# ut-amrl/vision_slam_frontend

Hardware: AMD Instinct MI355X
Metric: stereo frames/s (640x480, 2000 kp/frame) (higher is better)
Workload: dtype u8

## Files before the change

include/vsf.h:

```cpp
#ifndef VSF_H_
#define VSF_H_

#include <stddef.h>
#include <stdint.h>

#ifdef __cplusplus
extern "C" {
#endif

#define VSF_VERSION 2
#define VSF_DESC_BYTES 32
#define VSF_MAX_LEVELS 64

typedef enum {
  VSF_OK = 0,
  VSF_ERR_INVALID_ARG = 1,
  VSF_ERR_CAPACITY = 2,
  VSF_ERR_HIP = 3,
  VSF_ERR_UNSUPPORTED = 4,
  VSF_ERR_NO_DEVICE = 5
} vsf_status;

typedef struct {
  float x, y;
// ... 240 lines not shown


vsf_status vsf_debug_png_encode_header(int width, int height, int channels, uint8_t* out, size_t cap, size_t* n_bytes);
vsf_status vsf_debug_png_encode_cpu(const uint8_t* src, int width, int height, int channels, size_t src_row_stride, uint8_t* out,
                                    size_t cap, size_t* n_bytes);

vsf_status vsf_debug_jpeg_encode_header(int width, int height, int channels, int quality, uint8_t* out, size_t cap,
                                        size_t* n_bytes);

vsf_status vsf_debug_inject_hip_error(vsf_ctx* ctx, int code);
vsf_status vsf_debug_level_image(vsf_ctx* ctx, int image, int level, int blurred, uint8_t* out, size_t ostride);
vsf_status vsf_debug_fast_candidates(vsf_ctx* ctx, int image, int level, vsf_keypoint* kp_out, int cap,
                                     int* n_out);
vsf_status vsf_debug_fast_work(const vsf_params* p, int orb, int nms, uint32_t* words, int cap, int* n_words, int* n_full,
                               int32_t* levels_out, int level_cap);
vsf_status vsf_debug_level_keypoints(vsf_ctx* ctx, int image, int level, vsf_keypoint* kp_out, int cap,
                                     int* n_out);
vsf_status vsf_debug_retain_best(vsf_ctx* ctx, uint32_t* key_bits, uint32_t* ids, int n, int n_points, int use_lds,
                                 int mode, int* n_out);
vsf_status vsf_debug_sort_trim(vsf_ctx* ctx, const vsf_dmatch* matches, int n_lists, int n, float best_percent,
                               int serial, uint64_t* pairs_out, int32_t* counts_out);

vsf_status vsf_debug_jpeg_serial(vsf_ctx* ctx, int on);

#define VSF_STAGE_COUNT 8
enum { VSF_STAGE_PYRAMID = 0, VSF_STAGE_FAST, VSF_STAGE_SELECT, VSF_STAGE_BLUR, VSF_STAGE_DESCRIBE, VSF_STAGE_KNN2,
       VSF_STAGE_RATIO, VSF_STAGE_TAIL  };
vsf_status vsf_profile_enable(vsf_ctx* ctx, int on);
vsf_status vsf_profile_read(vsf_ctx* ctx, double* ms_total, int64_t* launches, int reset);
const char* vsf_stage_name(int stage);
// ... 9 lines not shown
```

vision_slam_frontend_amd/capi.py:

```python
from __future__ import annotations

import ctypes as C
from pathlib import Path

import numpy as np

_PKG = Path(__file__).resolve().parent
LIB_PATH = _PKG / "libvsf_hip.so"

KEYPOINT_DTYPE = np.dtype([("x", "<f4"), ("y", "<f4"), ("size", "<f4"), ("angle", "<f4"), ("response", "<f4"),
                           ("octave", "<i4"), ("class_id", "<i4")])
DMATCH_DTYPE = np.dtype([("queryIdx", "<i4"), ("trainIdx", "<i4"), ("imgIdx", "<i4"), ("distance", "<f4")])
VISION_FEATURE_DTYPE = np.dtype([("feature_idx", "<u8"), ("pixel", "<f4", (2,)), ("point3d", "<f4", (3,))])
FEATURE_MATCH_DTYPE = np.dtype([("feature_idx_initial", "<u8"), ("feature_idx_current", "<u8")])
assert VISION_FEATURE_DTYPE.itemsize == 28 and FEATURE_MATCH_DTYPE.itemsize == 16
DESC_BYTES = 32
PAYLOAD_MAGIC = 0x31465356

VSF_OK, VSF_ERR_INVALID_ARG, VSF_ERR_CAPACITY, VSF_ERR_HIP, VSF_ERR_UNSUPPORTED, VSF_ERR_NO_DEVICE = range(6)

EXPORTS = [
    "vsf_params_default", "vsf_params_set_ratio", "vsf_create", "vsf_destroy", "vsf_status_string",
    "vsf_last_hip_error", "vsf_get_params", "vsf_set_stream", "vsf_sync", "vsf_level_info", "vsf_extract",
    "vsf_fast_detect", "vsf_knn2_hamming", "vsf_get_matches", "vsf_extract_pair", "vsf_get_matches_multi", "vsf_extract_batch_dev", "vsf_match_batch_dev",
    "vsf_stereo_batch_dev", "vsf_set_lanes", "vsf_set_pipeline", "vsf_set_blur_overlap", "vsf_set_fast_resident", "vsf_get_fast_resident", "vsf_remove_ambig_stereo_batch_dev", "vsf_feature_matches_batch_dev", "vsf_bayer_bg_to_gray_batch_dev", "vsf_debug_level_image", "vsf_debug_fast_candidates", "vsf_debug_fast_work", "vsf_debug_level_keypoints",
    "vsf_algorithmic_bytes_per_image", "vsf_pyramid_pixels", "vsf_profile_enable", "vsf_profile_read",
    "vsf_stage_name", "vsf_debug_retain_best", "vsf_debug_sort_trim", "vsf_stereo_residuals_batch_dev", "vsf_stereo_thresholds_dev",
    "vsf_stereo_filter_batch_dev", "vsf_vision_features_batch_dev", "vsf_packed_outputs_capacity",
    "vsf_pack_outputs_dev", "vsf_observe_capacity", "vsf_observe_stereo", "vsf_observe_submit", "vsf_observe_collect", "vsf_observe_reset",
    "vsf_observe_configure", "vsf_observe_collect_view", "vsf_observe_stats", "vsf_observe_poll", "vsf_debug_jpeg_serial",
    "vsf_jpeg_decode_gray_batch", "vsf_png_decode_gray_batch", "vsf_imdecode_gray_batch", "vsf_tune_fast_resident", "vsf_set_option", "vsf_get_option", "vsf_debug_inject_hip_error", "vsf_comm_unique_id", "vsf_comm_create", "vsf_comm_destroy", "vsf_comm_info",
    "vsf_allgather_dev", "vsf_gather_payload_dev", "vsf_reserve", "vsf_set_input_event",
    "vsf_observe_set_debug_images", "vsf_observe_debug_view", "vsf_draw_canvases_dev", "vsf_draw_canvases",
    "vsf_observe_submit_compressed", "vsf_observe_stereo_compressed", "vsf_observe_set_compressed_cap",
    "vsf_observe_default_compressed_cap", "vsf_observe_compressed_slot_bytes", "vsf_observe_compressed_ring_bytes",
    "vsf_compressed_image_size", "vsf_observe_probe_compressed",
    "vsf_observe_set_debug_jpeg", "vsf_observe_debug_jpeg_view", "vsf_jpeg_encode_capacity", "vsf_jpeg_encode_batch_dev", "vsf_jpeg_encode", "vsf_debug_jpeg_encode_header",
    "vsf_png_encode_capacity", "vsf_png_encode_batch_dev", "vsf_png_encode", "vsf_debug_png_encode_header", "vsf_debug_png_encode_cpu", "vsf_observe_set_debug_png", "vsf_observe_debug_png_view",
]
(OPT_FAST_BOTH_MAX, OPT_SELECT_WIDE, OPT_PYRAMID_FEW, OPT_PYRAMID_CHAIN, OPT_PYRAMID_ROWS, OPT_SELECT_BIG_CLASS,
# ... 186 lines not shown
        L.vsf_observe_probe_compressed.argtypes = [vp, sz, i32, i32, sz, i32, ip]
        L.vsf_observe_set_debug_images.argtypes = [vp, i32]
        L.vsf_observe_debug_view.argtypes = [vp, C.c_int64, C.POINTER(vp), C.POINTER(vp)]
        L.vsf_observe_set_debug_jpeg.argtypes = [vp, i32]
        L.vsf_observe_debug_jpeg_view.argtypes = [vp, C.c_int64, C.POINTER(vp), C.POINTER(sz), C.POINTER(vp), C.POINTER(sz)]
        L.vsf_observe_set_debug_png.argtypes = [vp, i32]
        L.vsf_observe_debug_png_view.argtypes = [vp, C.c_int64, C.POINTER(vp), C.POINTER(sz), C.POINTER(vp), C.POINTER(sz)]
        L.vsf_draw_canvases_dev.argtypes = [vp, C.POINTER(VsfDrawCanvas), i32, vp, i32]
        L.vsf_draw_canvases.argtypes = [vp, C.POINTER(VsfDrawCanvas), i32, vp, i32]
        L.vsf_jpeg_decode_gray_batch.argtypes = [vp, vp, vp, i32, i32, i32, vp, sz, sz]
        L.vsf_png_decode_gray_batch.argtypes = [vp, vp, vp, i32, i32, i32, vp, sz, sz]
        L.vsf_imdecode_gray_batch.argtypes = [vp, vp, vp, i32, i32, i32, vp, sz, sz]
        L.vsf_debug_level_image.argtypes = [vp, i32, i32, i32, vp, sz]
        L.vsf_debug_fast_candidates.argtypes = [vp, i32, i32, vp, i32, ip]
        L.vsf_debug_fast_work.argtypes = [vp, i32, i32, vp, i32, ip, ip, vp, i32]
        L.vsf_debug_level_keypoints.argtypes = [vp, i32, i32, vp, i32, ip]
        L.vsf_algorithmic_bytes_per_image.argtypes = [vp]
        L.vsf_algorithmic_bytes_per_image.restype = C.c_uint64
        L.vsf_pyramid_pixels.argtypes = [vp]
        L.vsf_pyramid_pixels.restype = C.c_uint64
        L.vsf_debug_retain_best.argtypes = [vp, vp, vp, i32, i32, i32, i32, ip]
        L.vsf_profile_enable.argtypes = [vp, i32]
        L.vsf_profile_read.argtypes = [vp, C.POINTER(C.c_double), C.POINTER(C.c_int64), i32]
        L.vsf_stage_name.argtypes = [i32]
        L.vsf_stage_name.restype = C.c_char_p
        _lib = L
    return _lib


def _p(a):
# ... 518 lines not shown
```

vision_slam_frontend_amd/csrc/k_fast.hip:

```cpp
#include "vsf_gather.h"
#include <cstdlib>

#include "vsf_internal.h"

namespace {

typedef short v2s __attribute__((ext_vector_type(2)));
constexpr int SR = VSF_FAST_STRIP_ROWS;

struct FastArgs {
  const VsfLevel* levels;
  const uint32_t* units;
  int nwork_full;
  int nunits;
  const uint8_t* img0;
  size_t img0_stride;
  int img0_pitch;
  const uint8_t* pyr;
  uint32_t pyr_bytes;
  uint32_t* cand;
  uint32_t cand_entries;
  uint16_t* rowstart;
  int threshold;
  int nms;
};

__device__ __forceinline__ uint32_t wave_shr1(uint32_t v) {
  return (uint32_t)__builtin_amdgcn_update_dpp(0, (int)v, 0x138, 0xF, 0xF, true);
// ... 99 lines not shown

__device__ __forceinline__ ScoreRow make_score_row(v2s s02, v2s s13) {
  ScoreRow o;
  o.s02 = s02;
  o.s13 = s13;
  const v2s x = as_v2s(__builtin_amdgcn_alignbit(as_u32(s13), wave_shr1(as_u32(s13)), 16));
  const v2s y = as_v2s(__builtin_amdgcn_alignbit(wave_shl1(as_u32(s02)), as_u32(s02), 16));
  o.h2a = vmax(x, s13);
  o.h2b = vmax(s02, y);
  o.h3a = vmax3(x, s13, s02);
  o.h3b = vmax3(s02, y, s13);
  return o;
}

template <bool PACK, bool NMS>
__device__ __forceinline__ void fast_march_body(const FastArgs& a, int work, int image) {
  const int lane = threadIdx.x & 63;
  int level, band, strip, hl, nl, nrows0 = 0;
  bool valid = true, mixed = false, rim = false;
  VsfLevel L;
  if constexpr (PACK) {
    struct Item {
      uint32_t w[VSF_FAST_PACK_WORDS];
    };
    const Item P = uniform_copy(reinterpret_cast<const Item*>(a.units + a.nwork_full) + work);
    uint32_t w0 = P.w[4], w1 = P.w[5];
#pragma unroll
    for (int k = 1; k < VSF_FAST_PACK_SEGS; k++)
      if (k < (int)P.w[0] && lane >= (int)(P.w[5 + 2 * k] & 0xFFu)) w0 = P.w[4 + 2 * k], w1 = P.w[5 + 2 * k];
    nrows0 = (int)P.w[1];
    mixed = P.w[2] != 0u;
    rim = P.w[3] != 0u;
    level = (int)(w0 >> 24), band = (int)((w0 >> 16) & 0xFF), strip = (int)(w0 & 0x7FFF);
    hl = lane - (int)(w1 & 0xFFu);
    nl = (int)((w1 >> 8) & 0xFFu);
    valid = hl < nl;
    L = a.levels[level];
  } else {
    const uint32_t ud = uniform_copy(a.units + work);
    level = (int)(ud >> 24), band = (int)((ud >> 16) & 0xFF), strip = (int)(ud & 0x7FFF);
    L = uniform_copy(a.levels + level);
    hl = lane, nl = 64;
  }
  const int pitch = level == 0 ? a.img0_pitch : L.pitch, hrow = L.h;
  const uint8_t* src;
  uint32_t src_bytes;
  if constexpr (PACK) {
    const bool lvl0 = __builtin_amdgcn_readfirstlane(level) == 0;
    src = lvl0 ? a.img0 + (size_t)image * a.img0_stride : a.pyr + (size_t)image * a.pyr_bytes;
    src_bytes = lvl0 ? (uint32_t)(a.img0_pitch * __builtin_amdgcn_readfirstlane(hrow)) : a.pyr_bytes;
  } else {
    src = level == 0 ? a.img0 + (size_t)image * a.img0_stride : a.pyr + (size_t)image * a.pyr_bytes + L.offset;
    src_bytes = (uint32_t)(pitch * hrow);
  }
  const int t = a.threshold;
  const int offs = NMS ? max(t, 1) : t;
  const v2s toff = {(short)offs, (short)offs};
  const int bx0 = L.fast_a0 + VSF_FAST_BAND_COLS * band;
  const int c0 = bx0 - 4 + 4 * hl;
  const bool loadable = valid && c0 >= 0 && c0 + 3 < pitch;
  const int ys = L.y_lo + strip * SR;
  const int nrows = valid ? min(SR, L.y_hi - ys) : 0;
  if constexpr (!PACK) nrows0 = nrows;
  const int sx_lo = max(L.x_lo - 1, 3), sx_hi = min(L.x_hi + 1, L.w - 3);
  uint32_t sm02 = 0, sm13 = 0, em02 = 0, em13 = 0;
#pragma unroll
  for (int j = 0; j < 4; j++) {
    const int x = c0 + j;
    const uint32_t bit = 0xFFFFu << (16 * (j >> 1));
    const bool sc_ok = valid && ((hl >= 1 && hl <= nl - 2) || (hl == 0 && j == 3) || (hl == nl - 1 && j == 0)) &&
                       x >= sx_lo && x < sx_hi;
    const bool em_ok = valid && hl >= 1 && hl <= nl - 2 && x >= L.x_lo && x < L.x_hi && x < bx0 + VSF_FAST_BAND_COLS;
    if (j & 1) {
      if (sc_ok) sm13 |= bit;
      if (em_ok) em13 |= bit;
    } else {
      if (sc_ok) sm02 |= bit;
      if (em_ok) em02 |= bit;
    }
  }
  const int unit_local = strip * L.nbands + band;
  uint16_t* rs = a.rowstart + ((size_t)image * a.nunits + L.unit0 + unit_local) * VSF_FAST_RS_STRIDE;
  const int seg_cap = L.seg_cap;
  const __amdgpu_buffer_rsrc_t seg_rsrc =
      PACK ? __builtin_amdgcn_make_buffer_rsrc(a.cand + (size_t)image * a.cand_entries, 0, a.cand_entries * 4, 0x00020000)
           : __builtin_amdgcn_make_buffer_rsrc(a.cand + (size_t)image * a.cand_entries + L.cand_offset +
                                                   (size_t)unit_local * seg_cap,
                                               0, seg_cap * 4, 0x00020000);
  const uint32_t seg_off = PACK ? 4u * (L.cand_offset + (uint32_t)(unit_local * seg_cap)) : 0u;
  const __amdgpu_buffer_rsrc_t rs_rsrc = __builtin_amdgcn_make_buffer_rsrc(
      a.rowstart + (size_t)image * a.nunits * VSF_FAST_RS_STRIDE, 0, a.nunits * VSF_FAST_RS_STRIDE * 2, 0x00020000);
  const uint32_t rs_off = 2u * (uint32_t)((L.unit0 + unit_local) * VSF_FAST_RS_STRIDE);
  const bool rs_lane = PACK && valid && hl == 0;
  const int cfirst = lane - hl, cend = min(cfirst + nl, 64);
  const unsigned long long from_m = ~0ull << cfirst, cell_m = from_m & (cend >= 64 ? ~0ull : (1ull << cend) - 1ull);
  const uint32_t from_lo = (uint32_t)from_m, from_hi = (uint32_t)(from_m >> 32);
  const uint32_t cell_lo = (uint32_t)cell_m, cell_hi = (uint32_t)(cell_m >> 32);

  const __amdgpu_buffer_rsrc_t src_rsrc = __builtin_amdgcn_make_buffer_rsrc(const_cast<uint8_t*>(src), 0, src_bytes, 0x00020000);
  const uint32_t col_off = loadable ? (uint32_t)c0 : 0xFFFFFFF0u;
  const int qlo = 1 - ys, qhi = hrow - ys;
  const uint32_t rbase = loadable ? (level == 0 ? 0u : L.offset) + (uint32_t)(c0 + (ys - 1) * pitch) : 0x40000000u;
  auto load_row = [&](int q) -> uint32_t {
    if (PACK)
      return __builtin_amdgcn_raw_buffer_load_b32(src_rsrc, rbase + (uint32_t)__mul24(min(max(q, qlo), qhi), pitch), 0u,
                                                  0);
    const int yc = min(max(ys - 1 + q, 0), hrow - 1);
    return __builtin_amdgcn_raw_buffer_load_b32(src_rsrc, col_off, (uint32_t)(yc * pitch), 0);
// ... 2 lines not shown
  const unsigned long long scorable = __builtin_amdgcn_ballot_w64((sm02 | sm13) != 0u);
  const v2s zero2 = {0, 0};
  ScoreRow S0 = make_score_row(zero2, zero2), S1 = S0, S2 = S0;
  int count = 0;
  uint32_t my_rs = 0;
  const uint32_t yx0 = ((uint32_t)ys << 12) + (uint32_t)c0 + ((uint32_t)(NMS ? offs - 1 : 0) << 24);
  auto below = [&](unsigned long long b, int acc) -> int {
    if (PACK)
      return (int)__builtin_amdgcn_mbcnt_hi((uint32_t)(b >> 32) & from_hi,
                                            __builtin_amdgcn_mbcnt_lo((uint32_t)b & from_lo, (uint32_t)acc));
    return (int)__builtin_amdgcn_mbcnt_hi((uint32_t)(b >> 32), __builtin_amdgcn_mbcnt_lo((uint32_t)b, (uint32_t)acc));
  };
  auto in_cell = [&](unsigned long long b) -> int {
    if (PACK) return __popc((uint32_t)b & cell_lo) + __popc((uint32_t)(b >> 32) & cell_hi);
    return __popcll(b);
  };

  auto step = [&](int q, const RowP& R0, const RowP& R1, const RowP& R2, const RowP& R3, const RowP& R4,
                  const RowP& R5, RowP& R6, const ScoreRow& S_up, const ScoreRow& S_mid, ScoreRow& S_dn) {
    prep_row(R6);
    v2s s02 = zero2, s13 = zero2;
    const int sy = ys - 1 + q;
    const bool row_ok = sy >= 3 && sy < hrow - 3;
    const uint32_t far = max(__builtin_amdgcn_sad_u8(R0.d, R3.d, 0u), __builtin_amdgcn_sad_u8(R6.d, R3.d, 0u));
    unsigned long long want = __builtin_amdgcn_ballot_w64(far > (uint32_t)t) & scorable;
    if (PACK) {
      if (rim) want &= __builtin_amdgcn_ballot_w64(row_ok);
    } else {
      want &= row_ok ? ~0ull : 0ull;
    }
// ... 48 lines not shown
            if (k1) {
              if (!PACK || pos < seg_cap) __builtin_amdgcn_raw_buffer_store_b32(yx + 1, seg_rsrc, seg_off + 4u * (uint32_t)pos, 0, 0);
              ++pos;
            }
            if (k2) {
              if (!PACK || pos < seg_cap) __builtin_amdgcn_raw_buffer_store_b32(yx + 2, seg_rsrc, seg_off + 4u * (uint32_t)pos, 0, 0);
              ++pos;
            }
            if (k3) {
              if (!PACK || pos < seg_cap) __builtin_amdgcn_raw_buffer_store_b32(yx + 3, seg_rsrc, seg_off + 4u * (uint32_t)pos, 0, 0);
            }
            count += in_cell(b0) + in_cell(b1) + in_cell(b2) + in_cell(b3);
          }
        }
      }
      if (r + 1 < SR) {
        if (PACK) {
          if (rs_lane)
            __builtin_amdgcn_raw_buffer_store_b16((unsigned short)min(count, seg_cap), rs_rsrc, rs_off, 2u * (uint32_t)(r + 1), 0);
        } else {
          asm("s_mov_b32 m0, %2\n\ts_nop 0\n\tv_writelane_b32 %0, %1, m0" : "+v"(my_rs) : "s"(min(count, seg_cap)), "s"(r + 1));
        }
      }
    }
  };

  RowP A0, A1, A2, A3, A4, A5, A6, A7, A8;
  A0.d = load_row(-3), A1.d = load_row(-2), A2.d = load_row(-1), A3.d = load_row(0), A4.d = load_row(1), A5.d = load_row(2),
  A6.d = load_row(3), A7.d = load_row(4);
  prep_row(A0), prep_row(A1), prep_row(A2), prep_row(A3), prep_row(A4), prep_row(A5);
  const int qe = nrows0 + 1;
#define VSF_FAST_STEP(j, r0, r1, r2, r3, r4, r5, r6, ld, su, sm, sd) \
  if (q + (j) > qe) break;                                             \
  ld.d = load_row(q + (j) + 5);                                        \
  step(q + (j), r0, r1, r2, r3, r4, r5, r6, su, sm, sd);
  for (int q = 0;; q += 9) {
    VSF_FAST_STEP(0, A0, A1, A2, A3, A4, A5, A6, A8, S0, S1, S2)
    VSF_FAST_STEP(1, A1, A2, A3, A4, A5, A6, A7, A0, S1, S2, S0)
    VSF_FAST_STEP(2, A2, A3, A4, A5, A6, A7, A8, A1, S2, S0, S1)
    VSF_FAST_STEP(3, A3, A4, A5, A6, A7, A8, A0, A2, S0, S1, S2)
    VSF_FAST_STEP(4, A4, A5, A6, A7, A8, A0, A1, A3, S1, S2, S0)
    VSF_FAST_STEP(5, A5, A6, A7, A8, A0, A1, A2, A4, S2, S0, S1)
    VSF_FAST_STEP(6, A6, A7, A8, A0, A1, A2, A3, A5, S0, S1, S2)
    VSF_FAST_STEP(7, A7, A8, A0, A1, A2, A3, A4, A6, S1, S2, S0)
    VSF_FAST_STEP(8, A8, A0, A1, A2, A3, A4, A5, A7, S2, S0, S1)
  }
#undef VSF_FAST_STEP
  if (PACK) {
    if (rs_lane) {
      rs[0] = 0;
      rs[SR] = (uint16_t)min(count, seg_cap);
    }
  } else {
    if (hl < SR) rs[hl] = (uint16_t)my_rs;
    if (hl == 0) rs[SR] = (uint16_t)min(count, seg_cap);
  }
}

template <bool PACK, bool NMS>
__global__ __launch_bounds__(256) void fast_march_kernel(FastArgs a, int nwork) {
  const int item = __builtin_amdgcn_readfirstlane(blockIdx.x * 4 + (threadIdx.x >> 6));
  if (item >= nwork) return;
  fast_march_body<PACK, NMS>(a, item, blockIdx.y);
}

template <bool NMS>
__global__ __launch_bounds__(256) void fast_march_both_kernel(FastArgs a, int nfull, int npack) {
  const int item = __builtin_amdgcn_readfirstlane(blockIdx.x * 4 + (threadIdx.x >> 6));
  if (item >= nfull + npack) return;
  if (item < nfull)
    fast_march_body<false, NMS>(a, item, blockIdx.y);
  else
    fast_march_body<true, NMS>(a, item - nfull, blockIdx.y);
}

template <bool PACK, bool NMS>
__global__ __launch_bounds__(1024) void fast_march_resident_kernel(FastArgs a, int nwork, int nimages, uint32_t* next_cell) {
  const int total = nwork * nimages;
  while (true) {
    uint32_t r;
    asm volatile(
        "s_mov_b64 s[34:35], exec\n\t"
        "s_mov_b64 exec, 1\n\t"
        "global_atomic_add %0, %1, %2, %3 sc0\n\t"
        "s_waitcnt vmcnt(0)\n\t"
        "s_mov_b64 exec, s[34:35]"
        : "=&v"(r)
        : "v"(0u), "v"(1u), "s"(next_cell)
        : "memory", "s34", "s35");
    const uint32_t u = (uint32_t)__builtin_amdgcn_readfirstlane((int)r);
    if (u >= (uint32_t)total) break;
    const int image = (int)u / nwork, cell = (int)u - image * nwork;
    fast_march_body<PACK, NMS>(a, cell, image);
  }
}

__global__ __launch_bounds__(256) void fast_emit_kernel(const VsfLevel* __restrict__ levels,
                                                        const uint32_t* __restrict__ cand, uint32_t cand_entries,
                                                        const uint16_t* __restrict__ rowstart, int nunits,
                                                        int max_keypoints, vsf_keypoint* __restrict__ out,
                                                        int32_t* __restrict__ counts, int32_t* __restrict__ status) {
  __shared__ int cellpre[2048 + 8];
  __shared__ __attribute__((aligned(4))) uint16_t rs_lds[64 * VSF_FAST_RS_STRIDE];
  __shared__ int lds4[4];
  const int image = blockIdx.x;
  const VsfLevel L = levels[0];
  const uint16_t* rs_img = rowstart + (size_t)image * nunits * VSF_FAST_RS_STRIDE;
// ... 14 lines not shown
  });
  if (threadIdx.x == 0) {
    counts[image] = n;
    if (n > max_keypoints) atomicOr(status, 1);
  }
}

}

void vsf_launch_fast(const VsfDev& d, const VsfGeom& g, const VsfImages& im, int threshold, int nms, hipStream_t s,
                     int resident_waves_per_simd, int n_cus, uint32_t* d_cell_counters) {
  FastArgs a;
  a.levels = d.levels;
  a.units = d.units;
  a.nwork_full = g.nwork_full;
  a.nunits = g.nunits;
  a.img0 = im.base;
  a.img0_stride = im.image_stride;
  a.img0_pitch = (int)im.row_stride;
  a.pyr = d.pyr;
  a.pyr_bytes = g.pyr_bytes;
  a.cand = d.cand;
  a.cand_entries = g.cand_entries;
  a.rowstart = d.rowstart;
  a.threshold = threshold;
  a.nms = nms;
  if (resident_waves_per_simd > 0 && resident_waves_per_simd <= 4 && nms && d_cell_counters) {
    vsf_note(hipMemsetAsync(d_cell_counters, 0, 2 * sizeof(uint32_t), s));
    const dim3 block(256 * resident_waves_per_simd);
    if (g.nwork_full > 0)
      hipLaunchKernelGGL((fast_march_resident_kernel<false, true>), dim3(n_cus), block, 0, s, a, g.nwork_full, im.n,
                         d_cell_counters);
    if (g.nwork_pack > 0)
      hipLaunchKernelGGL((fast_march_resident_kernel<true, true>), dim3(n_cus), block, 0, s, a, g.nwork_pack, im.n,
                         d_cell_counters + 1);
    return;
  }
  const dim3 gf((g.nwork_full + 3) / 4, im.n), gp((g.nwork_pack + 3) / 4, im.n);
  const int both_max = d.tune ? d.tune->fast_both_max : 16;
  if (im.n <= both_max && g.nwork_full > 0 && g.nwork_pack > 0) {
    const dim3 gb((g.nwork_full + g.nwork_pack + 3) / 4, im.n);
    if (nms)
      hipLaunchKernelGGL((fast_march_both_kernel<true>), gb, dim3(256), 0, s, a, g.nwork_full, g.nwork_pack);
    else
      hipLaunchKernelGGL((fast_march_both_kernel<false>), gb, dim3(256), 0, s, a, g.nwork_full, g.nwork_pack);
    return;
  }
  if (nms) {
    if (g.nwork_full > 0) hipLaunchKernelGGL((fast_march_kernel<false, true>), gf, dim3(256), 0, s, a, g.nwork_full);
    if (g.nwork_pack > 0) hipLaunchKernelGGL((fast_march_kernel<true, true>), gp, dim3(256), 0, s, a, g.nwork_pack);
  } else {
    if (g.nwork_full > 0) hipLaunchKernelGGL((fast_march_kernel<false, false>), gf, dim3(256), 0, s, a, g.nwork_full);
    if (g.nwork_pack > 0) hipLaunchKernelGGL((fast_march_kernel<true, false>), gp, dim3(256), 0, s, a, g.nwork_pack);
  }
}

void vsf_launch_fast_emit(const VsfDev& d, const VsfGeom& g, int n_images, int max_keypoints, vsf_keypoint* d_kp,
                          int32_t* d_counts, hipStream_t s) {
  hipLaunchKernelGGL(fast_emit_kernel, dim3(n_images), dim3(256), 0, s, d.levels, d.cand, g.cand_entries, d.rowstart,
                     g.nunits, max_keypoints, d_kp, d_counts, d.status);
}
```

vision_slam_frontend_amd/csrc/vsf_api.hip:

```cpp
#include <algorithm>
#include <cfloat>
#include <climits>
#include <cmath>
#include <cstdio>
#include <cstring>
#include <new>
#include <vector>

#include "vsf_ctx.h"

using namespace vsfi;

thread_local int vsf_tls_hip_error = 0;

namespace vsfi {

vsf_status alloc_devset(vsf_ctx* ctx, const Geometry& G, DevSet* ds, bool orb, int n_images) {
  VSF_HIP(upload(&ds->levels, G.levels));
  VSF_HIP(upload(&ds->units, G.units));
  VSF_HIP(upload(&ds->blur_mma_units, G.blur_mma_units));
  VSF_HIP(upload(&ds->blur_mma_units_small, G.blur_mma_units_small));
  VSF_HIP(upload(&ds->blur_tcol, G.blur_tcol));
  VSF_HIP(upload(&ds->blur_tv, G.blur_tv));
  VSF_HIP(upload(&ds->ic_table, build_ic_table()));
  VsfDev& d = ds->d;
  d.ic_table = ds->ic_table;
  d.levels = ds->levels;
  d.units = ds->units;
  const size_t n = (size_t)n_images;
  if (orb) {
    VSF_HIP(hipMalloc((void**)&d.pyr, n * G.g.pyr_bytes));
    VSF_HIP(hipMalloc((void**)&d.blur, n * G.g.pyr_bytes));
    VSF_HIP(hipMalloc((void**)&d.scratch, n * 6 * G.g.cand_entries * sizeof(uint32_t)));
    VSF_HIP(hipMalloc((void**)&d.lvlkp, n * G.g.lvlkp_entries * sizeof(VsfLevelKp)));
    VSF_HIP(hipMalloc((void**)&d.lvl_count, n * G.g.nlevels * sizeof(int32_t)));
    VSF_HIP(hipMemset(d.lvl_count, 0, n * G.g.nlevels * sizeof(int32_t)));
  }
  VSF_HIP(hipMalloc((void**)&d.cand, n * G.g.cand_entries * sizeof(uint32_t)));
  const size_t rs_bytes = n * (size_t)std::max(G.g.nunits, 1) * VSF_FAST_RS_STRIDE * sizeof(uint16_t);
  VSF_HIP(hipMalloc((void**)&d.rowstart, rs_bytes));
  VSF_HIP(hipMemset(d.rowstart, 0, rs_bytes));
  d.status = ctx->d_status;
  d.tune = &ctx->tuning;
  ds->ready = true;
  return VSF_OK;
}

void free_devset(DevSet* ds) {
  hipFree(ds->levels);
  hipFree(ds->units);
  hipFree(ds->blur_mma_units);
  hipFree(ds->blur_mma_units_small);
  hipFree(ds->blur_tcol);
  hipFree(ds->blur_tv);
  hipFree(ds->ic_table);
  hipFree(ds->d.pyr);
  hipFree(ds->d.blur);
  hipFree(ds->d.scratch);
  hipFree(ds->d.lvlkp);
  hipFree(ds->d.lvl_count);
  hipFree(ds->d.cand);
  hipFree(ds->d.rowstart);
  *ds = DevSet();
}

// ... 701 lines not shown
```

vision_slam_frontend_amd/csrc/vsf_ctx.h:

```cpp
#ifndef VSF_CTX_H_
#define VSF_CTX_H_

#include <cstddef>
#include <cstdint>
#include <vector>

#include "vsf_internal.h"

namespace vsfi {

inline int align_up(int v, int a) { return (v + a - 1) / a * a; }

struct Geometry {
  VsfGeom g{};
  std::vector<VsfLevel> levels;
  std::vector<uint32_t> units;
  std::vector<VsfTap> xt, yt;
  std::vector<uint32_t> blur_mma_units, blur_mma_units_small;
  std::vector<uint4> blur_tcol, blur_tv;
  int blur_bias = 0;
};

struct DevSet {
  VsfDev d{};
  VsfLevel* levels = nullptr;
  uint32_t* units = nullptr;
  uint32_t* blur_mma_units = nullptr;
  uint32_t* blur_mma_units_small = nullptr;
  uint4* blur_tcol = nullptr;
  uint4* blur_tv = nullptr;
  uint2* ic_table = nullptr;
  bool ready = false;
};

bool build_geometry(const vsf_params& p, bool orb, bool nms, Geometry* out);
void gaussian_taps(int k[4]);
std::vector<uint2> build_ic_table();
std::vector<int> orb_umax(int patch_size);

}

// ... 329 lines not shown
```

vision_slam_frontend_amd/csrc/vsf_debug.hip:

```cpp
#include <algorithm>
#include <cfloat>
#include <climits>
#include <cmath>
#include <cstdio>
#include <cstring>
#include <new>
#include <vector>

#include "vsf_ctx.h"

using namespace vsfi;

extern "C" {

vsf_status vsf_debug_inject_hip_error(vsf_ctx* ctx, int code) {
  VsfErrorScope scope_(ctx);
  if (!ctx || code <= 0) return VSF_ERR_INVALID_ARG;
  vsf_note((hipError_t)code);
  return VSF_OK;
}

vsf_status vsf_debug_jpeg_serial(vsf_ctx* ctx, int on) {
  VsfErrorScope scope_(ctx);
  if (!ctx) return VSF_ERR_INVALID_ARG;
// ... 188 lines not shown
  Geometry G;
  if (!build_geometry(*p, orb != 0, nms != 0, &G)) return VSF_ERR_INVALID_ARG;
  const int n = G.g.nwork_full + G.g.nwork_pack * VSF_FAST_PACK_WORDS;
  *n_words = n;
  *n_full = G.g.nwork_full;
  for (int l = 0; l < (int)G.levels.size() && l < level_cap; l++) {
    const VsfLevel& L = G.levels[l];
    const int32_t v[10] = {L.w, L.h, L.x_lo, L.x_hi, L.y_lo, L.y_hi, L.fast_a0, L.nbands, L.nstrips, L.unit0};
    memcpy(levels_out + 10 * l, v, sizeof(v));
  }
  if (n > cap) return VSF_ERR_CAPACITY;
  if (n > 0) memcpy(words, G.units.data(), (size_t)n * sizeof(uint32_t));
  return VSF_OK;
}

vsf_status vsf_debug_level_keypoints(vsf_ctx* ctx, int image, int level, vsf_keypoint* kp_out, int cap, int* n_out) {
  VsfErrorScope scope_(ctx);
  if (!ctx || !n_out || !ctx->last_valid || image < 0 || image >= ctx->last_images.n || level < 0 ||
      level >= ctx->orb.g.nlevels)
    return VSF_ERR_INVALID_ARG;
  VSF_HIP(hipSetDevice(ctx->device));
  VSF_HIP(hipStreamSynchronize(ctx->stream));
  const VsfLevel& L = ctx->orb.levels[level];
  const VsfGeom& g = ctx->orb.g;
  int32_t n = 0;
  VSF_HIP(hipMemcpy(&n, ctx->dorb.d.lvl_count + (size_t)image * g.nlevels + level, sizeof(int32_t),
                    hipMemcpyDeviceToHost));
  std::vector<VsfLevelKp> v(std::max(n, 1));
  if (n > 0)
    VSF_HIP(hipMemcpy(v.data(), ctx->dorb.d.lvlkp + (size_t)image * g.lvlkp_entries + L.kp_offset,
// ... 10 lines not shown
```

vision_slam_frontend_amd/csrc/vsf_geometry.hip:

```cpp
#include <algorithm>
#include <cfloat>
#include <climits>
#include <cmath>
#include <cstdio>
#include <cstring>
#include <new>
#include <vector>

#include "vsf_ctx.h"

using namespace vsfi;

namespace {

inline int cvRoundD(double v) { return (int)std::nearbyint(v); }
inline int cvRoundF(float v) { return (int)std::nearbyintf(v); }
inline int cvFloorD(double v) {
  const int i = cvRoundD(v);
  return i - ((float)(v - i) < 0);
}
inline int cvCeilD(double v) {
  const int i = cvRoundD(v);
  return i + ((float)(i - v) < 0);
}
// ... 106 lines not shown
  for (int op = 0; op < 4; op++)
    for (int lane = 0; lane < 64; lane++) {
      const int n = lane & 31, h = lane >> 5, s = op & 1;
      uint16_t e[8];
      for (int j = 0; j < 8; j++) {
        const int row = 16 * s + 8 * (j >> 2) + 4 * h + (j & 3), d = row - n;
        const int tap = (n < VSF_BLUR_MMA_ROWS && d >= 0 && d < 7) ? k[d] : 0;
        e[j] = f16_bits_of_small_int(op >= 2 ? tap * 256 : tap);
      }
      uint4 v;
      memcpy(&v, e, 16);
      G->blur_tv.push_back(v);
    }
}

bool build_geometry(const vsf_params& p, bool orb, bool nms, Geometry* out) {
  Geometry& G = *out;
  const int nlevels = orb ? p.nlevels : 1;
  const int border = orb ? std::max(p.edge_threshold, 3) : 3;
  G.levels.assign(nlevels, VsfLevel{});
  G.g.nlevels = nlevels;
  G.g.width = p.width;
  G.g.height = p.height;
  const double scale_factor = (double)p.scale_factor;
  std::vector<int> nfeat(nlevels, 0);
  if (orb) {
    const float factor = (float)(1.0 / scale_factor);
    float nd = p.nfeatures * (1 - factor) / (1 - (float)std::pow((double)factor, (double)nlevels));
    int sum = 0;
    for (int l = 0; l < nlevels - 1; l++) {
// ... 107 lines not shown
      const VsfLevel& L = G.levels[c.level];
      mixed |= c.rows != c0.rows;
      rim |= L.y_lo - 1 < 3 || L.y_hi >= L.h - 3;
      w[4 + 2 * j] = ((uint32_t)c.level << 24) | ((uint32_t)c.band << 16) | (uint32_t)c.strip;
      w[5 + 2 * j] = (uint32_t)first | ((uint32_t)c.lanes << 8) | ((uint32_t)c.rows << 16);
      first += c.lanes;
    }
    w[2] = (uint32_t)mixed;
    w[3] = (uint32_t)rim;
    packs.insert(packs.end(), w, w + VSF_FAST_PACK_WORDS);
  }
  G.g.nwork_full = (int)G.units.size();
  G.g.nwork_pack = (int)(packs.size() / VSF_FAST_PACK_WORDS);
  G.units.insert(G.units.end(), packs.begin(), packs.end());
  if (G.units.empty()) G.units.push_back(0);
  G.g.lvlkp_entries = std::max(kp_off, 1);
  if (orb) {
    for (int l = 1; l < nlevels; l++) {
      VsfLevel& L = G.levels[l];
      const VsfLevel& P = G.levels[l - 1];
      L.xtab = (uint32_t)G.xt.size();
      L.ytab = (uint32_t)G.yt.size();
      build_taps(P.w, P.h, L.w, L.h, &G.xt, &G.yt);
      {
        const double sx = 1. / ((double)L.w / P.w), sy = 1. / ((double)L.h / P.h);
        memcpy(L.rscale_x, &sx, 8);
        memcpy(L.rscale_y, &sy, 8);
      }
      if (P.w < 8) return false;
      for (int x4 = 0; x4 < L.w; x4 += 4) {
// ... 84 lines not shown
```

vision_slam_frontend_amd/csrc/vsf_internal.h:

```cpp
#ifndef VSF_INTERNAL_H_
#define VSF_INTERNAL_H_

#include <hip/hip_runtime.h>
#include <stdint.h>

#include <vector>

#include "../../include/vsf.h"

#define VSF_FAST_BAND_COLS 248
#define VSF_FAST_PACK_SEGS 8
#define VSF_FAST_PACK_WORDS (4 + 2 * VSF_FAST_PACK_SEGS)
#define VSF_FAST_STRIP_ROWS 32
#define VSF_FAST_RS_STRIDE (VSF_FAST_STRIP_ROWS + 2)
#define VSF_BLUR_MMA_ROWS 26
#define VSF_BLUR_MMA_STEPS 16
#define VSF_BLUR_MMA_STEPS_SMALL 2
#define VSF_BLUR_TILE_OFFSET(pitch, x, y) \
  ((uint32_t)((y) >> 2) * (uint32_t)((pitch) * 4) + ((uint32_t)((x) >> 5) << 7) + ((uint32_t)((y) & 3) << 5) + (uint32_t)((x) & 31))
#define VSF_SORT_LDS_ROWS 4096
#define VSF_IC_ITEMS 320

struct VsfLevel {
  int32_t w, h;
  int32_t pitch;
  uint32_t offset;
  float scale;
  int32_t nfeatures;
// ... 26 lines not shown

struct VsfLevelKp {
  uint32_t xy;
  float response;
  float angle;
  float ca, sb;
};

struct VsfGeom {
  int nlevels;
  int width, height;
  uint32_t pyr_bytes;
  uint32_t cand_entries;
  int nunits;
  int nwork_full, nwork_pack;
  int lvlkp_entries;
  uint64_t pyramid_pixels;
};

struct VsfTuning {
  int fast_both_max = 16;
  int select_wide = 1;
  int pipe_priority = 0;
  int pipe_after_fast = 1;
  int select_big_class = 1;
  int jpeg_serial = 0;
  int pyramid_few = 16;
  int pyramid_chain = 8;
  int pyramid_rows = 6;
  int pyramid_tail_min = 0;
// ... 18 lines not shown
    if (ctx && enter) vsf_ctx_enter(ctx);
  }
  ~VsfErrorScope() {
    if (ctx && vsf_tls_hip_error != 0) vsf_ctx_absorb_noted_error(ctx);
  }
  VsfErrorScope(const VsfErrorScope&) = delete;
  VsfErrorScope& operator=(const VsfErrorScope&) = delete;
};
hipError_t vsf_prepare_sort_kernels(int lds_limit);
hipError_t vsf_prepare_pyramid_kernels(int lds_limit);
hipError_t vsf_prepare_jpeg_kernels(int lds_limit);

struct VsfDev {
  const VsfLevel* levels;
  const uint32_t* units;
  uint8_t* pyr;
  uint8_t* blur;
  uint32_t* cand;
  uint16_t* rowstart;
  uint32_t* scratch;
  VsfLevelKp* lvlkp;
  const uint2* ic_table;
  int32_t* lvl_count;
  int32_t* status;
  int status_stride;
  const VsfTuning* tune;
};

struct VsfImages {
  const uint8_t* base;
// ... 206 lines not shown
```

Measured before the change: 43020.

## Chain vertically adjacent FAST strips into one wave march

Adds a host-built chain table that groups up to four vertically consecutive FAST strip cells (both full and packed work items) so a single wave marches through them continuously. Row-start and candidate segment pointers are advanced at each strip seam instead of ending the wave. This avoids reloading the halo rows at each strip boundary and cuts per-item setup cost. In exchange there are fewer, longer work items, sorted longest first, which can reduce parallelism and load balance on small levels.

Result: slower. 42370 (-1.5%).

```diff
diff --git a/include/vsf.h b/include/vsf.h
--- a/include/vsf.h
+++ b/include/vsf.h
@@ -278,6 +278,8 @@
                                      int* n_out);
 vsf_status vsf_debug_fast_work(const vsf_params* p, int orb, int nms, uint32_t* words, int cap, int* n_words, int* n_full,
                                int32_t* levels_out, int level_cap);
+vsf_status vsf_debug_fast_chains(const vsf_params* p, int orb, int nms, int32_t* items, int item_cap, int* n_items,
+                                 int32_t* chain_begin, int chain_cap, int* n_chains, int* n_full_chains, int* chain_max);
 vsf_status vsf_debug_level_keypoints(vsf_ctx* ctx, int image, int level, vsf_keypoint* kp_out, int cap,
                                      int* n_out);
 vsf_status vsf_debug_retain_best(vsf_ctx* ctx, uint32_t* key_bits, uint32_t* ids, int n, int n_points, int use_lds,
diff --git a/vision_slam_frontend_amd/capi.py b/vision_slam_frontend_amd/capi.py
--- a/vision_slam_frontend_amd/capi.py
+++ b/vision_slam_frontend_amd/capi.py
@@ -23,7 +23,7 @@
     "vsf_params_default", "vsf_params_set_ratio", "vsf_create", "vsf_destroy", "vsf_status_string",
     "vsf_last_hip_error", "vsf_get_params", "vsf_set_stream", "vsf_sync", "vsf_level_info", "vsf_extract",
     "vsf_fast_detect", "vsf_knn2_hamming", "vsf_get_matches", "vsf_extract_pair", "vsf_get_matches_multi", "vsf_extract_batch_dev", "vsf_match_batch_dev",
-    "vsf_stereo_batch_dev", "vsf_set_lanes", "vsf_set_pipeline", "vsf_set_blur_overlap", "vsf_set_fast_resident", "vsf_get_fast_resident", "vsf_remove_ambig_stereo_batch_dev", "vsf_feature_matches_batch_dev", "vsf_bayer_bg_to_gray_batch_dev", "vsf_debug_level_image", "vsf_debug_fast_candidates", "vsf_debug_fast_work", "vsf_debug_level_keypoints",
+    "vsf_stereo_batch_dev", "vsf_set_lanes", "vsf_set_pipeline", "vsf_set_blur_overlap", "vsf_set_fast_resident", "vsf_get_fast_resident", "vsf_remove_ambig_stereo_batch_dev", "vsf_feature_matches_batch_dev", "vsf_bayer_bg_to_gray_batch_dev", "vsf_debug_level_image", "vsf_debug_fast_candidates", "vsf_debug_fast_work", "vsf_debug_fast_chains", "vsf_debug_level_keypoints",
     "vsf_algorithmic_bytes_per_image", "vsf_pyramid_pixels", "vsf_profile_enable", "vsf_profile_read",
     "vsf_stage_name", "vsf_debug_retain_best", "vsf_debug_sort_trim", "vsf_stereo_residuals_batch_dev", "vsf_stereo_thresholds_dev",
     "vsf_stereo_filter_batch_dev", "vsf_vision_features_batch_dev", "vsf_packed_outputs_capacity",
@@ -240,6 +240,7 @@
         L.vsf_debug_level_image.argtypes = [vp, i32, i32, i32, vp, sz]
         L.vsf_debug_fast_candidates.argtypes = [vp, i32, i32, vp, i32, ip]
         L.vsf_debug_fast_work.argtypes = [vp, i32, i32, vp, i32, ip, ip, vp, i32]
+        L.vsf_debug_fast_chains.argtypes = [vp, i32, i32, vp, i32, ip, vp, i32, ip, ip, ip]
         L.vsf_debug_level_keypoints.argtypes = [vp, i32, i32, vp, i32, ip]
         L.vsf_algorithmic_bytes_per_image.argtypes = [vp]
         L.vsf_algorithmic_bytes_per_image.restype = C.c_uint64
diff --git a/vision_slam_frontend_amd/csrc/k_fast.hip b/vision_slam_frontend_amd/csrc/k_fast.hip
--- a/vision_slam_frontend_amd/csrc/k_fast.hip
+++ b/vision_slam_frontend_amd/csrc/k_fast.hip
@@ -12,6 +12,8 @@
   const VsfLevel* levels;
   const uint32_t* units;
   int nwork_full;
+  const uint32_t* chains;
+  int nchain_full;
   int nunits;
   const uint8_t* img0;
   size_t img0_stride;
@@ -141,10 +143,12 @@
 }
 
 template <bool PACK, bool NMS>
-__device__ __forceinline__ void fast_march_body(const FastArgs& a, int work, int image) {
+__device__ __forceinline__ void fast_march_body(const FastArgs& a, int chain, int image) {
   const int lane = threadIdx.x & 63;
-  int level, band, strip, hl, nl, nrows0 = 0;
-  bool valid = true, mixed = false, rim = false;
+  const uint32_t cw = uniform_copy(a.chains + (PACK ? a.nchain_full : 0) + chain);
+  const int work = (int)(cw >> 12), nrows0 = (int)(cw & 0xFFFu);
+  int level, band, strip, hl, nl;
+  bool valid = true, rim = false;
   VsfLevel L;
   if constexpr (PACK) {
     struct Item {
@@ -155,8 +159,6 @@
 #pragma unroll
     for (int k = 1; k < VSF_FAST_PACK_SEGS; k++)
       if (k < (int)P.w[0] && lane >= (int)(P.w[5 + 2 * k] & 0xFFu)) w0 = P.w[4 + 2 * k], w1 = P.w[5 + 2 * k];
-    nrows0 = (int)P.w[1];
-    mixed = P.w[2] != 0u;
     rim = P.w[3] != 0u;
     level = (int)(w0 >> 24), band = (int)((w0 >> 16) & 0xFF), strip = (int)(w0 & 0x7FFF);
     hl = lane - (int)(w1 & 0xFFu);
@@ -187,8 +189,8 @@
   const int c0 = bx0 - 4 + 4 * hl;
   const bool loadable = valid && c0 >= 0 && c0 + 3 < pitch;
   const int ys = L.y_lo + strip * SR;
-  const int nrows = valid ? min(SR, L.y_hi - ys) : 0;
-  if constexpr (!PACK) nrows0 = nrows;
+  const int nrows = valid ? min(nrows0, L.y_hi - ys) : 0;
+  const bool mixed = PACK && __builtin_amdgcn_ballot_w64(valid && nrows != nrows0) != 0ull;
   const int sx_lo = max(L.x_lo - 1, 3), sx_hi = min(L.x_hi + 1, L.w - 3);
   uint32_t sm02 = 0, sm13 = 0, em02 = 0, em13 = 0;
 #pragma unroll
@@ -208,17 +210,15 @@
   }
   const int unit_local = strip * L.nbands + band;
   uint16_t* rs = a.rowstart + ((size_t)image * a.nunits + L.unit0 + unit_local) * VSF_FAST_RS_STRIDE;
-  const int seg_cap = L.seg_cap;
-  const __amdgpu_buffer_rsrc_t seg_rsrc =
-      PACK ? __builtin_amdgcn_make_buffer_rsrc(a.cand + (size_t)image * a.cand_entries, 0, a.cand_entries * 4, 0x00020000)
-           : __builtin_amdgcn_make_buffer_rsrc(a.cand + (size_t)image * a.cand_entries + L.cand_offset +
-                                                   (size_t)unit_local * seg_cap,
-                                               0, seg_cap * 4, 0x00020000);
-  const uint32_t seg_off = PACK ? 4u * (L.cand_offset + (uint32_t)(unit_local * seg_cap)) : 0u;
+  const int seg_cap = L.seg_cap, seam_units = L.nbands;
+  uint32_t* seg_ptr = a.cand + (size_t)image * a.cand_entries + (PACK ? (size_t)0 : L.cand_offset + (size_t)unit_local * seg_cap);
+  __amdgpu_buffer_rsrc_t seg_rsrc =
+      __builtin_amdgcn_make_buffer_rsrc(seg_ptr, 0, (PACK ? (int)a.cand_entries : seg_cap) * 4, 0x00020000);
+  uint32_t seg_off = PACK ? 4u * (L.cand_offset + (uint32_t)(unit_local * seg_cap)) : 0u;
   const __amdgpu_buffer_rsrc_t rs_rsrc = __builtin_amdgcn_make_buffer_rsrc(
       a.rowstart + (size_t)image * a.nunits * VSF_FAST_RS_STRIDE, 0, a.nunits * VSF_FAST_RS_STRIDE * 2, 0x00020000);
-  const uint32_t rs_off = 2u * (uint32_t)((L.unit0 + unit_local) * VSF_FAST_RS_STRIDE);
-  const bool rs_lane = PACK && valid && hl == 0;
+  uint32_t rs_off = 2u * (uint32_t)((L.unit0 + unit_local) * VSF_FAST_RS_STRIDE);
+  bool rs_lane = PACK && valid && hl == 0;
   const int cfirst = lane - hl, cend = min(cfirst + nl, 64);
   const unsigned long long from_m = ~0ull << cfirst, cell_m = from_m & (cend >= 64 ? ~0ull : (1ull << cend) - 1ull);
   const uint32_t from_lo = (uint32_t)from_m, from_hi = (uint32_t)(from_m >> 32);
@@ -251,6 +251,18 @@
   auto in_cell = [&](unsigned long long b) -> int {
     if (PACK) return __popc((uint32_t)b & cell_lo) + __popc((uint32_t)(b >> 32) & cell_hi);
     return __popcll(b);
+  };
+
+  auto finish_cell = [&]() {
+    if (PACK) {
+      if (rs_lane) {
+        __builtin_amdgcn_raw_buffer_store_b16((unsigned short)0, rs_rsrc, rs_off, 0u, 0);
+        __builtin_amdgcn_raw_buffer_store_b16((unsigned short)min(count, seg_cap), rs_rsrc, rs_off, 2u * (uint32_t)SR, 0);
+      }
+    } else {
+      if (hl < SR) rs[hl] = (uint16_t)my_rs;
+      if (hl == 0) rs[SR] = (uint16_t)min(count, seg_cap);
+    }
   };
 
   auto step = [&](int q, const RowP& R0, const RowP& R1, const RowP& R2, const RowP& R3, const RowP& R4,
@@ -329,13 +341,27 @@
           }
         }
       }
-      if (r + 1 < SR) {
+      const int lr = r & (SR - 1);
+      if (lr + 1 < SR) {
         if (PACK) {
           if (rs_lane)
-            __builtin_amdgcn_raw_buffer_store_b16((unsigned short)min(count, seg_cap), rs_rsrc, rs_off, 2u * (uint32_t)(r + 1), 0);
+            __builtin_amdgcn_raw_buffer_store_b16((unsigned short)min(count, seg_cap), rs_rsrc, rs_off, 2u * (uint32_t)(lr + 1), 0);
         } else {
-          asm("s_mov_b32 m0, %2\n\ts_nop 0\n\tv_writelane_b32 %0, %1, m0" : "+v"(my_rs) : "s"(min(count, seg_cap)), "s"(r + 1));
+          asm("s_mov_b32 m0, %2\n\ts_nop 0\n\tv_writelane_b32 %0, %1, m0" : "+v"(my_rs) : "s"(min(count, seg_cap)), "s"(lr + 1));
         }
+      } else if (r + 1 < nrows0) {
+        finish_cell();
+        if (PACK) {
+          rs_lane = rs_lane && r + 1 < nrows;
+          rs_off += 2u * (uint32_t)(seam_units * VSF_FAST_RS_STRIDE);
+          seg_off += 4u * (uint32_t)(seam_units * seg_cap);
+        } else {
+          rs += seam_units * VSF_FAST_RS_STRIDE;
+          seg_ptr += seam_units * seg_cap;
+          seg_rsrc = __builtin_amdgcn_make_buffer_rsrc(seg_ptr, 0, seg_cap * 4, 0x00020000);
+          my_rs = 0;
+        }
+        count = 0;
       }
     }
   };
@@ -361,21 +387,13 @@
     VSF_FAST_STEP(8, A8, A0, A1, A2, A3, A4, A5, A7, S2, S0, S1)
   }
 #undef VSF_FAST_STEP
-  if (PACK) {
-    if (rs_lane) {
-      rs[0] = 0;
-      rs[SR] = (uint16_t)min(count, seg_cap);
-    }
-  } else {
-    if (hl < SR) rs[hl] = (uint16_t)my_rs;
-    if (hl == 0) rs[SR] = (uint16_t)min(count, seg_cap);
-  }
+  finish_cell();
 }
 
 template <bool PACK, bool NMS>
-__global__ __launch_bounds__(256) void fast_march_kernel(FastArgs a, int nwork) {
+__global__ __launch_bounds__(256) void fast_march_kernel(FastArgs a, int nchains) {
   const int item = __builtin_amdgcn_readfirstlane(blockIdx.x * 4 + (threadIdx.x >> 6));
-  if (item >= nwork) return;
+  if (item >= nchains) return;
   fast_march_body<PACK, NMS>(a, item, blockIdx.y);
 }
 
@@ -390,8 +408,8 @@
 }
 
 template <bool PACK, bool NMS>
-__global__ __launch_bounds__(1024) void fast_march_resident_kernel(FastArgs a, int nwork, int nimages, uint32_t* next_cell) {
-  const int total = nwork * nimages;
+__global__ __launch_bounds__(1024) void fast_march_resident_kernel(FastArgs a, int nchains, int nimages, uint32_t* next_cell) {
+  const int total = nchains * nimages;
   while (true) {
     uint32_t r;
     asm volatile(
@@ -405,7 +423,7 @@
         : "memory", "s34", "s35");
     const uint32_t u = (uint32_t)__builtin_amdgcn_readfirstlane((int)r);
     if (u >= (uint32_t)total) break;
-    const int image = (int)u / nwork, cell = (int)u - image * nwork;
+    const int image = (int)u / nchains, cell = (int)u - image * nchains;
     fast_march_body<PACK, NMS>(a, cell, image);
   }
 }
@@ -450,6 +468,8 @@
   a.levels = d.levels;
   a.units = d.units;
   a.nwork_full = g.nwork_full;
+  a.chains = d.chains;
+  a.nchain_full = g.nchain_full;
   a.nunits = g.nunits;
   a.img0 = im.base;
   a.img0_stride = im.image_stride;
@@ -464,30 +484,30 @@
   if (resident_waves_per_simd > 0 && resident_waves_per_simd <= 4 && nms && d_cell_counters) {
     vsf_note(hipMemsetAsync(d_cell_counters, 0, 2 * sizeof(uint32_t), s));
     const dim3 block(256 * resident_waves_per_simd);
-    if (g.nwork_full > 0)
-      hipLaunchKernelGGL((fast_march_resident_kernel<false, true>), dim3(n_cus), block, 0, s, a, g.nwork_full, im.n,
+    if (g.nchain_full > 0)
+      hipLaunchKernelGGL((fast_march_resident_kernel<false, true>), dim3(n_cus), block, 0, s, a, g.nchain_full, im.n,
                          d_cell_counters);
-    if (g.nwork_pack > 0)
-      hipLaunchKernelGGL((fast_march_resident_kernel<true, true>), dim3(n_cus), block, 0, s, a, g.nwork_pack, im.n,
+    if (g.nchain_pack > 0)
+      hipLaunchKernelGGL((fast_march_resident_kernel<true, true>), dim3(n_cus), block, 0, s, a, g.nchain_pack, im.n,
                          d_cell_counters + 1);
     return;
   }
-  const dim3 gf((g.nwork_full + 3) / 4, im.n), gp((g.nwork_pack + 3) / 4, im.n);
+  const dim3 gf((g.nchain_full + 3) / 4, im.n), gp((g.nchain_pack + 3) / 4, im.n);
   const int both_max = d.tune ? d.tune->fast_both_max : 16;
-  if (im.n <= both_max && g.nwork_full > 0 && g.nwork_pack > 0) {
-    const dim3 gb((g.nwork_full + g.nwork_pack + 3) / 4, im.n);
+  if (im.n <= both_max && g.nchain_full > 0 && g.nchain_pack > 0) {
+    const dim3 gb((g.nchain_full + g.nchain_pack + 3) / 4, im.n);
     if (nms)
-      hipLaunchKernelGGL((fast_march_both_kernel<true>), gb, dim3(256), 0, s, a, g.nwork_full, g.nwork_pack);
+      hipLaunchKernelGGL((fast_march_both_kernel<true>), gb, dim3(256), 0, s, a, g.nchain_full, g.nchain_pack);
     else
-      hipLaunchKernelGGL((fast_march_both_kernel<false>), gb, dim3(256), 0, s, a, g.nwork_full, g.nwork_pack);
+      hipLaunchKernelGGL((fast_march_both_kernel<false>), gb, dim3(256), 0, s, a, g.nchain_full, g.nchain_pack);
     return;
   }
   if (nms) {
-    if (g.nwork_full > 0) hipLaunchKernelGGL((fast_march_kernel<false, true>), gf, dim3(256), 0, s, a, g.nwork_full);
-    if (g.nwork_pack > 0) hipLaunchKernelGGL((fast_march_kernel<true, true>), gp, dim3(256), 0, s, a, g.nwork_pack);
+    if (g.nchain_full > 0) hipLaunchKernelGGL((fast_march_kernel<false, true>), gf, dim3(256), 0, s, a, g.nchain_full);
+    if (g.nchain_pack > 0) hipLaunchKernelGGL((fast_march_kernel<true, true>), gp, dim3(256), 0, s, a, g.nchain_pack);
   } else {
-    if (g.nwork_full > 0) hipLaunchKernelGGL((fast_march_kernel<false, false>), gf, dim3(256), 0, s, a, g.nwork_full);
-    if (g.nwork_pack > 0) hipLaunchKernelGGL((fast_march_kernel<true, false>), gp, dim3(256), 0, s, a, g.nwork_pack);
+    if (g.nchain_full > 0) hipLaunchKernelGGL((fast_march_kernel<false, false>), gf, dim3(256), 0, s, a, g.nchain_full);
+    if (g.nchain_pack > 0) hipLaunchKernelGGL((fast_march_kernel<true, false>), gp, dim3(256), 0, s, a, g.nchain_pack);
   }
 }
 
diff --git a/vision_slam_frontend_amd/csrc/vsf_api.hip b/vision_slam_frontend_amd/csrc/vsf_api.hip
--- a/vision_slam_frontend_amd/csrc/vsf_api.hip
+++ b/vision_slam_frontend_amd/csrc/vsf_api.hip
@@ -18,6 +18,7 @@
 vsf_status alloc_devset(vsf_ctx* ctx, const Geometry& G, DevSet* ds, bool orb, int n_images) {
   VSF_HIP(upload(&ds->levels, G.levels));
   VSF_HIP(upload(&ds->units, G.units));
+  VSF_HIP(upload(&ds->chains, G.chains));
   VSF_HIP(upload(&ds->blur_mma_units, G.blur_mma_units));
   VSF_HIP(upload(&ds->blur_mma_units_small, G.blur_mma_units_small));
   VSF_HIP(upload(&ds->blur_tcol, G.blur_tcol));
@@ -27,6 +28,7 @@
   d.ic_table = ds->ic_table;
   d.levels = ds->levels;
   d.units = ds->units;
+  d.chains = ds->chains;
   const size_t n = (size_t)n_images;
   if (orb) {
     VSF_HIP(hipMalloc((void**)&d.pyr, n * G.g.pyr_bytes));
@@ -49,6 +51,7 @@
 void free_devset(DevSet* ds) {
   hipFree(ds->levels);
   hipFree(ds->units);
+  hipFree(ds->chains);
   hipFree(ds->blur_mma_units);
   hipFree(ds->blur_mma_units_small);
   hipFree(ds->blur_tcol);
diff --git a/vision_slam_frontend_amd/csrc/vsf_ctx.h b/vision_slam_frontend_amd/csrc/vsf_ctx.h
--- a/vision_slam_frontend_amd/csrc/vsf_ctx.h
+++ b/vision_slam_frontend_amd/csrc/vsf_ctx.h
@@ -15,6 +15,8 @@
   VsfGeom g{};
   std::vector<VsfLevel> levels;
   std::vector<uint32_t> units;
+  std::vector<uint32_t> chains;
+  std::vector<int> chain_items, chain_begin;
   std::vector<VsfTap> xt, yt;
   std::vector<uint32_t> blur_mma_units, blur_mma_units_small;
   std::vector<uint4> blur_tcol, blur_tv;
@@ -25,6 +27,7 @@
   VsfDev d{};
   VsfLevel* levels = nullptr;
   uint32_t* units = nullptr;
+  uint32_t* chains = nullptr;
   uint32_t* blur_mma_units = nullptr;
   uint32_t* blur_mma_units_small = nullptr;
   uint4* blur_tcol = nullptr;
diff --git a/vision_slam_frontend_amd/csrc/vsf_debug.hip b/vision_slam_frontend_amd/csrc/vsf_debug.hip
--- a/vision_slam_frontend_amd/csrc/vsf_debug.hip
+++ b/vision_slam_frontend_amd/csrc/vsf_debug.hip
@@ -226,6 +226,27 @@
   return VSF_OK;
 }
 
+vsf_status vsf_debug_fast_chains(const vsf_params* p, int orb, int nms, int32_t* items, int item_cap, int* n_items,
+                                 int32_t* chain_begin, int chain_cap, int* n_chains, int* n_full_chains, int* chain_max) {
+  if (!p || !n_items || !n_chains || !n_full_chains || item_cap < 0 || chain_cap < 0 || (item_cap > 0 && !items) ||
+      (chain_cap > 0 && !chain_begin))
+    return VSF_ERR_INVALID_ARG;
+  if (p->nlevels < 1 || p->nlevels > VSF_MAX_LEVELS || p->width < 16 || p->height < 16 || !(p->scale_factor > 1.0f) ||
+      p->edge_threshold < 0 || p->first_level != 0)
+    return VSF_ERR_INVALID_ARG;
+  Geometry G;
+  if (!build_geometry(*p, orb != 0, nms != 0, &G)) return VSF_ERR_INVALID_ARG;
+  const int nc = G.g.nchain_full + G.g.nchain_pack, ni = (int)G.chain_items.size();
+  *n_items = ni;
+  *n_chains = nc;
+  *n_full_chains = G.g.nchain_full;
+  if (chain_max) *chain_max = VSF_FAST_CHAIN_MAX;
+  if (ni > item_cap || nc + 1 > chain_cap) return VSF_ERR_CAPACITY;
+  if (ni > 0) memcpy(items, G.chain_items.data(), (size_t)ni * sizeof(int32_t));
+  memcpy(chain_begin, G.chain_begin.data(), (size_t)(nc + 1) * sizeof(int32_t));
+  return VSF_OK;
+}
+
 vsf_status vsf_debug_level_keypoints(vsf_ctx* ctx, int image, int level, vsf_keypoint* kp_out, int cap, int* n_out) {
   VsfErrorScope scope_(ctx);
   if (!ctx || !n_out || !ctx->last_valid || image < 0 || image >= ctx->last_images.n || level < 0 ||
diff --git a/vision_slam_frontend_amd/csrc/vsf_geometry.hip b/vision_slam_frontend_amd/csrc/vsf_geometry.hip
--- a/vision_slam_frontend_amd/csrc/vsf_geometry.hip
+++ b/vision_slam_frontend_amd/csrc/vsf_geometry.hip
@@ -144,6 +144,100 @@
     }
 }
 
+bool build_fast_chains(Geometry* out) {
+  Geometry& G = *out;
+  const int nfull = G.g.nwork_full, npack = G.g.nwork_pack;
+  struct Chain {
+    int first, rows;
+  };
+  G.chain_items.clear();
+  G.chain_begin.clear();
+  std::vector<Chain> chains[2];
+  std::vector<std::vector<int>> members[2];
+  auto cut = [&](int kind, const std::vector<int>& run, const std::vector<int>& rows) {
+    const int n = (int)run.size(), nch = (n + VSF_FAST_CHAIN_MAX - 1) / VSF_FAST_CHAIN_MAX;
+    for (int c = 0, i = 0; c < nch; c++) {
+      const int len = n / nch + (c < n % nch ? 1 : 0);
+      int total = 0;
+      for (int j = 0; j < len; j++) total += rows[i + j];
+      chains[kind].push_back(Chain{run[i], total});
+      members[kind].push_back(std::vector<int>(run.begin() + i, run.begin() + i + len));
+      i += len;
+    }
+  };
+  auto cell_rows = [&](uint32_t w0) {
+    const VsfLevel& L = G.levels[w0 >> 24];
+    return std::min(VSF_FAST_STRIP_ROWS, L.y_hi - (L.y_lo + VSF_FAST_STRIP_ROWS * (int)(w0 & 0x7FFF)));
+  };
+  {
+    std::vector<int> order(nfull);
+    for (int i = 0; i < nfull; i++) order[i] = i;
+    std::stable_sort(order.begin(), order.end(), [&](int a, int b) { return G.units[a] < G.units[b]; });
+    std::vector<int> run, rows;
+    for (int k = 0; k < nfull; k++) {
+      const uint32_t w = G.units[order[k]];
+      if (!run.empty() && w != G.units[run.back()] + 1u) {
+        cut(0, run, rows);
+        run.clear(), rows.clear();
+      }
+      run.push_back(order[k]);
+      rows.push_back(cell_rows(w));
+    }
+    if (!run.empty()) cut(0, run, rows);
+  }
+  {
+    const uint32_t* P = G.units.data() + nfull;
+    std::vector<int> succ(npack, -1);
+    std::vector<char> has_pred(npack, 0);
+    for (int ia = 0; ia < npack; ia++) {
+      const uint32_t* A = P + (size_t)ia * VSF_FAST_PACK_WORDS;
+      if (A[1] != (uint32_t)VSF_FAST_STRIP_ROWS || A[2] != 0u) continue;
+      for (int ib = 0; ib < npack; ib++) {
+        const uint32_t* B = P + (size_t)ib * VSF_FAST_PACK_WORDS;
+        if (B[4] != A[4] + 1u || B[0] > A[0] || B[3] != A[3] || has_pred[ib]) continue;
+        bool ok = true;
+        for (uint32_t j = 0; j < A[0] && ok; j++) {
+          if (j < B[0])
+            ok = B[4 + 2 * j] == A[4 + 2 * j] + 1u && (B[5 + 2 * j] & 0xFFFFu) == (A[5 + 2 * j] & 0xFFFFu);
+          else
+            ok = (int)(A[4 + 2 * j] & 0x7FFF) + 1 >= G.levels[A[4 + 2 * j] >> 24].nstrips;
+        }
+        if (ok) {
+          succ[ia] = ib;
+          has_pred[ib] = 1;
+          break;
+        }
+      }
+    }
+    for (int i0 = 0; i0 < npack; i0++) {
+      if (has_pred[i0]) continue;
+      std::vector<int> run, rows;
+      for (int i = i0; i >= 0; i = succ[i]) {
+        run.push_back(i);
+        rows.push_back((int)P[(size_t)i * VSF_FAST_PACK_WORDS + 1]);
+      }
+      cut(1, run, rows);
+    }
+  }
+  G.chains.clear();
+  for (int kind = 0; kind < 2; kind++) {
+    std::vector<int> order(chains[kind].size());
+    for (size_t i = 0; i < order.size(); i++) order[i] = (int)i;
+    std::stable_sort(order.begin(), order.end(), [&](int a, int b) { return chains[kind][a].rows > chains[kind][b].rows; });
+    for (int c : order) {
+      const Chain& ch = chains[kind][c];
+      if (ch.first >= (1 << 20) || ch.rows > 0xFFF) return false;
+      G.chains.push_back(((uint32_t)ch.first << 12) | (uint32_t)ch.rows);
+      G.chain_begin.push_back((int)G.chain_items.size());
+      for (int it : members[kind][c]) G.chain_items.push_back(kind == 0 ? it : nfull + it);
+    }
+    (kind == 0 ? G.g.nchain_full : G.g.nchain_pack) = (int)order.size();
+  }
+  G.chain_begin.push_back((int)G.chain_items.size());
+  if (G.chains.empty()) G.chains.push_back(0);
+  return true;
+}
+
 bool build_geometry(const vsf_params& p, bool orb, bool nms, Geometry* out) {
   Geometry& G = *out;
   const int nlevels = orb ? p.nlevels : 1;
@@ -281,6 +375,7 @@
   G.g.nwork_pack = (int)(packs.size() / VSF_FAST_PACK_WORDS);
   G.units.insert(G.units.end(), packs.begin(), packs.end());
   if (G.units.empty()) G.units.push_back(0);
+  if (!build_fast_chains(&G)) return false;
   G.g.lvlkp_entries = std::max(kp_off, 1);
   if (orb) {
     for (int l = 1; l < nlevels; l++) {
diff --git a/vision_slam_frontend_amd/csrc/vsf_internal.h b/vision_slam_frontend_amd/csrc/vsf_internal.h
--- a/vision_slam_frontend_amd/csrc/vsf_internal.h
+++ b/vision_slam_frontend_amd/csrc/vsf_internal.h
@@ -12,6 +12,9 @@
 #define VSF_FAST_PACK_SEGS 8
 #define VSF_FAST_PACK_WORDS (4 + 2 * VSF_FAST_PACK_SEGS)
 #define VSF_FAST_STRIP_ROWS 32
+#ifndef VSF_FAST_CHAIN_MAX
+#define VSF_FAST_CHAIN_MAX 4
+#endif
 #define VSF_FAST_RS_STRIDE (VSF_FAST_STRIP_ROWS + 2)
 #define VSF_BLUR_MMA_ROWS 26
 #define VSF_BLUR_MMA_STEPS 16
@@ -68,6 +71,7 @@
   uint32_t cand_entries;
   int nunits;
   int nwork_full, nwork_pack;
+  int nchain_full, nchain_pack;
   int lvlkp_entries;
   uint64_t pyramid_pixels;
 };
@@ -116,6 +120,7 @@
 struct VsfDev {
   const VsfLevel* levels;
   const uint32_t* units;
+  const uint32_t* chains;
   uint8_t* pyr;
   uint8_t* blur;
   uint32_t* cand;
```
